# prip-lab/MSU-LatentAFIS

Hardware: AMD Instinct MI355X
Metric: latent queries/sec vs 100k rolled gallery (higher is better)
Workload: dtype f32

## Files before the change

### msu-latentafis_amd/csrc/graph.hip

```cpp
#include "afis_device.h"
#include <type_traits>
#include "atan2f_libm.h"
#include "graph_arith.h"
#include "stdsort_order.h"

namespace afis {

#define AFIS_PI 3.1415926

#if defined(AFIS_PHASE_TIMING) && !defined(AFIS_GRAPH_PAIRS_UNIT)
__device__ u64 g_graph_phase[16];
#define GPH_INIT() u64 gph_t0 = __builtin_readcyclecounter()
#define GPH(i) do { if (threadIdx.x == 0) { const u64 t1_ = __builtin_readcyclecounter(); sm.ph[(i)] += t1_ - gph_t0; gph_t0 = t1_; } } while (0)
#define GPH_T0() const u64 gph_k0 = __builtin_readcyclecounter()
#define GPH_K(i) do { if (threadIdx.x == 0) sm.ph[(i)] += __builtin_readcyclecounter() - gph_k0; } while (0)
#define GPH_ZERO() do { if (threadIdx.x < 16) sm.ph[threadIdx.x] = 0; WSYNC(); } while (0)
#define GPH_FLUSH() do { WSYNC(); if (threadIdx.x < 16 && sm.ph[threadIdx.x]) atomicAdd(&g_graph_phase[threadIdx.x], sm.ph[threadIdx.x]); } while (0)
#else
#define GPH_INIT() do {} while (0)
#define GPH(i) do {} while (0)
#define GPH_T0() do {} while (0)
#define GPH_K(i) do {} while (0)
#define GPH_ZERO() do {} while (0)
#define GPH_FLUSH() do {} while (0)
#endif

__device__ __forceinline__ u64 g_make_key(float v, int idx) { return rank_composite(rank_key(v), (uint32_t)idx); }
__device__ __forceinline__ int g_wave_popc(bool p) { return __popcll(__ballot(p)); }
__device__ __forceinline__ int g_lane_prefix(u64 mask) { return __builtin_amdgcn_mbcnt_hi((uint32_t)(mask >> 32), __builtin_amdgcn_mbcnt_lo((uint32_t)mask, 0)); }
#define WSYNC() __syncthreads()

__device__ __forceinline__ int g_wave_max(int x)
{
    x = max(x, __builtin_amdgcn_update_dpp(0, x, 0xB1, 0xf, 0xf, false));
    x = max(x, __builtin_amdgcn_update_dpp(0, x, 0x4E, 0xf, 0xf, false));
    x = max(x, __builtin_amdgcn_update_dpp(0, x, 0x124, 0xf, 0xf, false));
    x = max(x, __builtin_amdgcn_update_dpp(0, x, 0x128, 0xf, 0xf, false));
    x = max(x, __builtin_amdgcn_update_dpp(x, x, 0x142, 0xa, 0xf, false));
    x = max(x, __builtin_amdgcn_update_dpp(x, x, 0x143, 0xc, 0xf, false));
    return __builtin_amdgcn_readlane(x, 63);
}

__device__ __forceinline__ uint32_t g_wave_max_u32(uint32_t x) { return (uint32_t)g_wave_max((int)(x ^ 0x80000000u)) ^ 0x80000000u; }
__device__ __forceinline__ uint32_t g_wave_min_u32(uint32_t x) { return ~g_wave_max_u32(~x); }

__device__ __forceinline__ int g_wave_sum(int x)
{
    x += __builtin_amdgcn_update_dpp(0, x, 0xB1, 0xf, 0xf, false);
    x += __builtin_amdgcn_update_dpp(0, x, 0x4E, 0xf, 0xf, false);
    x += __builtin_amdgcn_update_dpp(0, x, 0x124, 0xf, 0xf, false);
    x += __builtin_amdgcn_update_dpp(0, x, 0x128, 0xf, 0xf, false);
    x += __builtin_amdgcn_update_dpp(0, x, 0x142, 0xa, 0xf, false);
    x += __builtin_amdgcn_update_dpp(0, x, 0x143, 0xc, 0xf, false);
    return __builtin_amdgcn_readlane(x, 63);
}

typedef __amdgpu_buffer_rsrc_t SlabBuf;
typedef uint32_t v4u __attribute__((ext_vector_type(4)));
__device__ __forceinline__ SlabBuf g_slab_buf(unsigned char* base, uint32_t bytes) { return __builtin_amdgcn_make_buffer_rsrc(base, 0, (int)bytes, 0x00020000); }

struct Pt { int lx, ly, rx, ry; };
__device__ __forceinline__ int2 pack_xy(int lx, int ly, int rx, int ry) { return make_int2((lx & 0xffff) | (ly << 16), (rx & 0xffff) | (ry << 16)); }
__device__ __forceinline__ Pt unpack_xy(int2 v) { Pt p; p.lx = (int)(short)v.x; p.ly = v.x >> 16; p.rx = (int)(short)v.y; p.ry = v.y >> 16; return p; }

template <int N, bool OWN> struct SimStore { float simv[N]; };
template <int N> struct SimStore<N, false> {};

#ifndef AFIS_MINU_ALIAS
#define AFIS_MINU_ALIAS 1
#endif
constexpr int kSortShort = 48;
template <int NMAX_, bool OWN_SIM_>
struct __attribute__((aligned(16))) WaveSmem : SimStore<NMAX_, OWN_SIM_> {
    static constexpr int NMAX = NMAX_;
    static constexpr bool OWN_SIM = OWN_SIM_;
    static constexpr bool ALIAS_ORI = NMAX_ > 128 || AFIS_MINU_ALIAS;
    static constexpr int W = (NMAX + 31) / 32;
    static constexpr int N4 = (NMAX + 3) / 4 * 4;
    static constexpr int U = (NMAX + 63) / 64;
    float b[N4];
    union {
        float cc[N4];
        struct { short order[NMAX]; short sel[NMAX]; } os;
    } y;
    short li[NMAX], ri[NMAX];
    int2 xy[NMAX];
    union {
        uint32_t hb[NMAX][W];
        struct { uint32_t keys[N4]; short te[NMAX], targ[NMAX]; } pick;
        uint32_t s7key[NMAX > 128 ? 256 : 1];
    };
    union {
        uint32_t cnt[128];
        u64 keys[kSortShort];
        struct { float lo[ALIAS_ORI ? 1 : NMAX], ro[ALIAS_ORI ? 1 : NMAX]; } s;
    } x;
#ifdef AFIS_PHASE_TIMING
    u64 ph[16];
#endif
};
template <class SM> __device__ __forceinline__ int l_row(int v) { if constexpr (SM::OWN_SIM) return v; else return v & 1023; }
template <class SM> __device__ __forceinline__ int r_pt(int v) { if constexpr (SM::OWN_SIM) return v; else return v & 1023; }
__device__ __forceinline__ int tex_slot_of(int li, int ri) { return ((li >> 10) & 31) | (((ri >> 10) & 31) << 5); }
__device__ __forceinline__ short tex_pack_l(int row, int slot) { return (short)(row | ((slot & 31) << 10)); }
__device__ __forceinline__ short tex_pack_r(int pt, int slot) { return (short)(pt | ((slot >> 5) << 10)); }
template <class SM>
__device__ __forceinline__ float list_sim(const SM& sm, const float* __restrict__ ext, int t)
{
    if constexpr (SM::OWN_SIM) return sm.simv[t];
    else return ext[tex_slot_of(sm.li[t], sm.ri[t])];
}

__device__ __forceinline__ int next_task(int32_t* ctr)
{
    int t;
    unsigned long long saved;
    asm volatile("s_mov_b64 %1, exec\n\t"
                 "s_mov_b64 exec, 1\n\t"
                 "global_atomic_add %0, %2, %3, %4 sc0\n\t"
                 "s_waitcnt vmcnt(0)\n\t"
                 "s_mov_b64 exec, %1"
                 : "=&v"(t), "=&s"(saved) : "v"(0), "v"(1), "s"(ctr) : "memory");
    return __builtin_amdgcn_readfirstlane(t);
}

template <class SM, int ref_tie>
__device__ __forceinline__ void sort_scores(SM& sm, int num, double thr)
{
    const int lane = threadIdx.x;
    constexpr int U = SM::U;
    uint32_t* const s_cnt = sm.x.cnt;
    uint32_t* const s_gkey = reinterpret_cast<uint32_t*>(sm.y.cc);
    uint32_t* const s_key = s_gkey;
    uint32_t m32[U]; int r[U];
    if (num <= kSortShort) {
        const u64 mine = lane < num ? g_make_key(sm.b[lane], lane) : 0ull;
        if (lane < num) sm.x.keys[lane] = mine;
        WSYNC();
        int rr = 0;
        for (int k = 0; k < num; ++k) rr += sm.x.keys[k] > mine;
        if (ref_tie && num > 16) {
            int gg = 0;
            for (int k = 0; k < num; ++k) gg += (uint32_t)(sm.x.keys[k] >> 32) > (uint32_t)(mine >> 32);
            const bool tied = lane < num && gg != rr && !((double)sm.b[lane] < thr);
            if (__ballot(tied) != 0ull) {
                constexpr int kOrd = kSortShort / 2;
                uint32_t* const k32 = s_gkey + kOrd;
                static_assert(SM::N4 >= kOrd + 2 * kSortShort, "no room in cc for the keys and the stack of the std::sort restatement");
                WSYNC();
                if (lane < num) { k32[lane] = (uint32_t)(mine >> 32); sm.y.os.order[lane] = (short)lane; }
                WSYNC();
                if (lane == 0) stdsort_prefix<uint16_t>(reinterpret_cast<uint16_t*>(sm.y.os.order), num, num, k32, reinterpret_cast<int*>(k32 + kSortShort));
                WSYNC();
                return;
            }
        }
        WSYNC();
        if (lane < num) sm.y.os.order[rr] = (short)lane;
        WSYNC();
        return;
    }
    uint32_t kmin = 0xffffffffu, kmax = 0u;
#pragma unroll
    for (int u = 0; u < U; ++u) {
        const int t = lane + 64 * u;
        m32[u] = t < num ? rank_key(sm.b[t]) : 0u;
        if (t < num) { kmin = min(kmin, m32[u]); kmax = max(kmax, m32[u]); }
    }
#pragma unroll
    for (int off = 32; off >= 1; off >>= 1) { kmin = min(kmin, (uint32_t)__shfl_xor((int)kmin, off)); kmax = max(kmax, (uint32_t)__shfl_xor((int)kmax, off)); }
    const uint32_t span = kmax - kmin;
    const int sh = max(0, 26 - __clz((int)(span | 1u)));
    int bin[U];
// ... 150 lines not shown
    if (LOOKUP) {
        const int dx1 = abs(a.lx - o.lx), dx2 = abs(a.rx - o.rx), dy1 = abs(a.ly - o.ly), dy2 = abs(a.ry - o.ry);
        ok = !((dx1 >= kDistN) | (dx2 >= kDistN) | (dy1 >= kDistN) | (dy2 >= kDistN));
        d1 = sqrt_rn_pos((float)(256 * (dx1 * dx1 + dy1 * dy1)));
        d2 = sqrt_rn_pos((float)(256 * (dx2 * dx2 + dy2 * dy2)));
        (void)table;
    } else {
        const float dx1 = (float)(a.lx - o.lx), dx2 = (float)(a.rx - o.rx), dy1 = (float)(a.ly - o.ly), dy2 = (float)(a.ry - o.ry);
        const float p = dx1 * dx1, q = dy1 * dy1, r = dx2 * dx2, s = dy2 * dy2;
        d1 = sqrt_rn_pos(p + q);
        d2 = sqrt_rn_pos(r + s);
    }
    dist = fabsf(d1 - d2);
    return ok;
}
template <bool LOOKUP>
__device__ __forceinline__ bool pair_compatible(const Pt& a, const Pt& o, const float* __restrict__ table)
{
    float s1, s2; bool ok = true;
    if (LOOKUP) {
        const int dx1 = abs(a.lx - o.lx), dx2 = abs(a.rx - o.rx), dy1 = abs(a.ly - o.ly), dy2 = abs(a.ry - o.ry);
        ok = !((dx1 >= kDistN) | (dx2 >= kDistN) | (dy1 >= kDistN) | (dy2 >= kDistN));
        s1 = (float)(256 * (dx1 * dx1 + dy1 * dy1)); s2 = (float)(256 * (dx2 * dx2 + dy2 * dy2));
    } else {
        const float dx1 = (float)(a.lx - o.lx), dx2 = (float)(a.rx - o.rx), dy1 = (float)(a.ly - o.ly), dy2 = (float)(a.ry - o.ry);
        const float p = dx1 * dx1, q = dy1 * dy1, r = dx2 * dx2, s = dy2 * dy2;
        s1 = p + q; s2 = r + s;
    }
    const float d1 = __builtin_amdgcn_sqrtf(s1), d2 = __builtin_amdgcn_sqrtf(s2);
    const float dist = fabsf(d1 - d2);
    const float slack = fmaxf(d1, d2) * 4.76837158e-7f;
    if (fabsf(dist - 30.0f) > slack) return ok && dist < 30.0f;
    float exact;
    pair_dist<LOOKUP>(a, o, table, exact);
    return ok && exact < 30.0f;
}
template <bool RANGE_TEST>
__device__ __forceinline__ bool tex_pair_dist(int2 a, int2 o, float& dist)
{
    float n1, n2;
    pair_n(a, o, n1, n2);
    dist = 16.0f * fabsf(sqrt_rn_int(n1) - sqrt_rn_int(n2));
    return RANGE_TEST ? tex_in_range(a, o) : true;
}
template <bool RANGE_TEST>
__device__ __forceinline__ bool tex_pair_compatible(int2 a, int2 o)
{
    float n1, n2;
    pair_n(a, o, n1, n2);
    const bool ok = RANGE_TEST ? tex_in_range(a, o) : true;
    return pair_compatible_n<true>(n1, n2) && ok;
}

__device__ __forceinline__ float minu_pair_dist(int2 a, int2 o)
{
    float n1, n2;
    pair_n(a, o, n1, n2);
    return fabsf(sqrt_rn_int(n1) - sqrt_rn_int(n2));
}
__device__ __forceinline__ bool minu_pair_compatible(int2 a, int2 o)
{
    float n1, n2;
    pair_n(a, o, n1, n2);
    return pair_compatible_n<false>(n1, n2);
}

__device__ __forceinline__ float h_of_x(float x)
{
    const float q0 = x * 0.04f;
    const float r = fmaf(-q0, 25.0f, x);
    const float h = fmaf(r, 0.04f, q0);
    return __builtin_amdgcn_fmed3f(h, 0.0f, 1.0f);
}
__device__ __forceinline__ float h_value(float dist)
{
    const float x = 30.0f - dist;
    const float q0 = x * 0.04f;
    const float r = fmaf(-q0, 25.0f, x);
    const float h = fmaf(r, 0.04f, q0);
    return __builtin_amdgcn_fmed3f(h, 0.0f, 1.0f);
}

template <class SM, bool LOOKUP, int ITERS, int MODE, int REF_TIE>
__device__ int dist_filter(SM& sm, int num, const float* __restrict__ table, const float* __restrict__ ext, SlabBuf slab)
{
    constexpr bool fast = MODE > 0;
    constexpr bool range_test = MODE == 1;
    auto compat_fast = [](int2 a, int2 o) -> bool { if (LOOKUP) return tex_pair_compatible<range_test>(a, o); return minu_pair_compatible(a, o); };
    auto dist_fast = [](int2 a, int2 o) -> float { float d; if (LOOKUP) { tex_pair_dist<range_test>(a, o, d); return d; } return minu_pair_dist(a, o); };
    constexpr int U = SM::U, W = SM::W, NMAX = SM::NMAX;
    [[maybe_unused]] constexpr int PH = LOOKUP ? 8 : 0;
    GPH_INIT();
    const int lane = threadIdx.x;
    for (int i = lane; i < num * W; i += 64) sm.hb[i / W][i % W] = 0u;
    int2 me[U];
#pragma unroll
    for (int u = 0; u < U; ++u) {
        const int t = lane + 64 * u;
        if (t < SM::N4) { sm.b[t] = t < num ? list_sim(sm, ext, t) : 0.0f; sm.y.cc[t] = 0.0f; }
        me[u] = t < num ? sm.xy[t] : make_int2(0, 0);
    }
    WSYNC();
    const int half = num >> 1;
    const bool even = !(num & 1);
    uint32_t* const hb0 = &sm.hb[0][0];
    auto pair = [&](int2 own, int t, int k, int2 other) {
        if (fast ? compat_fast(own, other) : pair_compatible<LOOKUP>(unpack_xy(own), unpack_xy(other), table)) {
            atomicOr(hb0 + (t * W + (k >> 5)), 1u << (k & 31));
            atomicOr(hb0 + (__umul24(k, W) + (t >> 5)), 1u << (t & 31));
        }
    };
    const int tail0 = num & ~63, R = num - tail0;
    const bool grouped = R > 0 && R <= 32;
    const int n_wide = grouped ? tail0 : num;
    uint32_t kb[U];
    const uint32_t num8 = (uint32_t)num * 8u;
#pragma unroll
    for (int u = 0; u < U; ++u) { const int t = lane + 64 * u; kb[u] = t < num ? (uint32_t)t * 8u : 0u; }
#ifndef AFIS_PAIR_UNROLL
#define AFIS_PAIR_UNROLL 1
#endif
    constexpr int DU = fast ? AFIS_PAIR_UNROLL : 1;
    auto pair_loop = [&](auto ua_tag) {
    constexpr int UA = decltype(ua_tag)::value;
    for (int d = 1; d <= half; d += DU) {
        int2 other[DU][UA];
        int kk[DU][UA];
#pragma unroll
        for (int s2 = 0; s2 < DU; ++s2) {
#pragma unroll
            for (int u = 0; u < UA; ++u) {
                const uint32_t a = kb[u] + 8u;
                kb[u] = min(a, a - num8);
                other[s2][u] = *reinterpret_cast<const int2*>(reinterpret_cast<const char*>(sm.xy) + kb[u]);
                kk[s2][u] = (int)(kb[u] >> 3);
            }
        }
        __builtin_amdgcn_sched_barrier(0);
        if (fast) {
            float n1[DU][UA], n2[DU][UA]; bool hit[DU][UA], near[DU][UA]; bool any_near = false;
#pragma unroll
            for (int s2 = 0; s2 < DU; ++s2) {
#pragma unroll
                for (int u = 0; u < UA; ++u) {
                    pair_n(me[u], other[s2][u], n1[s2][u], n2[s2][u]);
                    hit[s2][u] = pair_compatible_t<LOOKUP>(n1[s2][u], n2[s2][u], near[s2][u]);
                    hit[s2][u] = hit[s2][u] | near[s2][u];
                }
            }
            (void)any_near;
#pragma unroll
            for (int s2 = 0; s2 < DU; ++s2) {
                const bool last = d + s2 == half && even;
#pragma unroll
                for (int u = 0; u < UA; ++u) {
                    const int t = lane + 64 * u, k = kk[s2][u];
                    bool ok = hit[s2][u] && t < n_wide && d + s2 <= half && !(last && t >= half);
                    if (LOOKUP && range_test) ok = ok && tex_in_range(me[u], other[s2][u]);
                    if constexpr (LOOKUP) {
                        const int ts = t < num ? t : 0;
                        atomicOr(hb0 + (ts * W + (k >> 5)), ok ? 1u << (k & 31) : 0u);
                        atomicOr(hb0 + (__umul24(k, W) + (ts >> 5)), ok ? 1u << (ts & 31) : 0u);
                    } else if (ok) {
                        atomicOr(hb0 + (t * W + (k >> 5)), 1u << (k & 31));
                        atomicOr(hb0 + (__umul24(k, W) + (t >> 5)), 1u << (t & 31));
                    }
                }
            }
        } else {
            const bool last = d == half && even;
#pragma unroll
            for (int u = 0; u < UA; ++u) {
                const int t = lane + 64 * u;
                if (t < n_wide && !(last && t >= half)) pair(me[u], t, kk[0][u], other[0][u]);
            }
        }
    }
    };
    const int n_blk = (n_wide + 63) >> 6;
    if (n_blk >= U) pair_loop(std::integral_constant<int, U>{});
    else if (U > 1 && n_blk == U - 1) pair_loop(std::integral_constant<int, (U > 1 ? U - 1 : 1)>{});
    else if (n_blk > 0) pair_loop(std::integral_constant<int, U>{});
    if (grouped) {
        const int sh = R <= 8 ? 3 : R <= 16 ? 4 : 5, RG = 1 << sh, dstep = 64 >> sh;
        const int r = lane & (RG - 1), t = tail0 + r;
        const bool row = r < R;
        const int2 own = row ? sm.xy[t] : make_int2(0, 0);
        int d = 1 + (lane >> sh);
        int k = t + d; k = k >= num ? k - num : k;
        for (int d0 = 1; d0 <= half; d0 += dstep) {
            if (row && d <= half && !(d == half && even && t >= half)) pair(own, t, k, sm.xy[k]);
            d += dstep; k += dstep; k = k >= num ? k - num : k;
        }
    }
    WSYNC();
    GPH(PH + 0);
    int myrow[U], trip[U], rlen[U];
    const int Wn = (num + 31) / 32;
    {
        int cnt[U];
#pragma unroll
        for (int u = 0; u < U; ++u) {
            const int t = lane + 64 * u;
            int c = -1;
            if (t < num) {
                c = 0; for (int w = 0; w < Wn; ++w) c += __popc(sm.hb[t][w]);
                sm.y.os.sel[t] = (short)c;
                c = min(c >> 2, 15);
            }
            cnt[u] = c;
        }
        int base = 0;
        for (int bk = 15; bk >= 0; --bk) {
#pragma unroll
            for (int u = 0; u < U; ++u) {
                const bool in = cnt[u] == bk;
                const u64 m = __ballot(in);
                if (in) sm.y.os.order[base + g_lane_prefix(m)] = (short)(lane + 64 * u);
                base += __popcll(m);
            }
        }
        WSYNC();
#pragma unroll
        for (int u = 0; u < U; ++u) {
            const int p = lane + 64 * u;
            myrow[u] = p < num ? (int)sm.y.os.order[p] : -1;
            rlen[u] = myrow[u] >= 0 ? (int)sm.y.os.sel[myrow[u]] : 0;
            trip[u] = g_wave_max(rlen[u]);
        }
        WSYNC();
        for (int t = num + lane; t < SM::N4; t += 64) sm.y.cc[t] = 0.0f;
    }
    int2 mine[U];
#pragma unroll
    for (int u = 0; u < U; ++u) mine[u] = myrow[u] >= 0 ? sm.xy[myrow[u]] : make_int2(0, 0);
    constexpr bool kFlat = NMAX > 128;
    constexpr int kSlabN = kFlat ? kTexSlabSteps : kMinuSlabSteps;
    static_assert(kSlabN % 4 == 0, "the read loop takes blocks of four steps");
    static_assert((size_t)U * kSlabN * 64 * 5 == (kFlat ? kTexSlabWgBytes : kMinuSlabWgBytes), "slab layout and the size the host allocates differ");
    constexpr int kSlabBlk = kSlabN / 4;
    constexpr uint32_t kSlabIdx0 = (uint32_t)U * kSlabN * 64 * 4;
    const uint32_t lane16 = (uint32_t)lane * 16u, lane4 = (uint32_t)lane * 4u;
    auto put_block = [&](int e, const float (&h)[4], uint32_t k4) {
        __builtin_amdgcn_raw_buffer_store_b128(v4u{__float_as_uint(h[0]), __float_as_uint(h[1]), __float_as_uint(h[2]), __float_as_uint(h[3])}, slab, lane16, e * 1024, 0);
        __builtin_amdgcn_raw_buffer_store_b32(k4, slab, lane4, (int)kSlabIdx0 + e * 256, 0);
    };
    auto get_block = [&](int e, v4u& h, uint32_t& k4) {
        h = __builtin_amdgcn_raw_buffer_load_b128(slab, lane16, e * 1024, 0);
        k4 = __builtin_amdgcn_raw_buffer_load_b32(slab, lane4, (int)kSlabIdx0 + e * 256, 0);
    };
    int cur_w[U]; uint32_t cur_bits[U];
#pragma unroll
    for (int u = 0; u < U; ++u) { cur_w[u] = 0; cur_bits[u] = 0u; }
    auto value = [&](int2 own, int k) -> float {
        float dist;
        if (fast && LOOKUP) {
            float n1, n2;
            pair_n(own, sm.xy[k], n1, n2);
            return h_of_x(fmaf(-16.0f, fabsf(sqrt_rn_int(n1) - sqrt_rn_int(n2)), 30.0f));
        }
        if (fast) dist = dist_fast(own, sm.xy[k]);
        else pair_dist<LOOKUP>(unpack_xy(own), unpack_xy(sm.xy[k]), table, dist);
        return h_value(dist);
    };
    for (int it = 0; it < ITERS; ++it) {
#pragma unroll
        for (int u = 0; u < U; ++u) {
            const int t = myrow[u];
            const uint32_t* hrow = sm.hb[t >= 0 ? t : 0];
            float acc = 0.0f;
            if (it == 0) {
                if (t >= 0) {
                    int w = 0;
                    uint32_t bits = hrow[0];
                    for (int n0 = 0; n0 < trip[u]; n0 += 4) {
                        if (n0 == kSlabN) { cur_w[u] = w; cur_bits[u] = bits; }
                        float h4[4] = {0.0f, 0.0f, 0.0f, 0.0f};
                        uint32_t k4 = 0u;
#pragma unroll
                        for (int j = 0; j < 4; ++j) {
                            if (n0 + j < trip[u]) {
                                while (bits == 0u && w + 1 < Wn) { ++w; bits = hrow[w]; }
                                const bool have = bits != 0u;
                                const int k = (w * 32 + __ffs(bits) - 1) & 255;
                                bits &= bits - 1;
                                const float h = value(mine[u], k);
                                h4[j] = h; k4 |= (uint32_t)k << (8 * j);
                                const float p = h * sm.b[k];
                                acc += have ? p : 0.0f;
                            }
                        }
                        if (n0 < kSlabN) put_block(u * kSlabBlk + (n0 >> 2), h4, k4);
                    }
                }
            } else {
                const int nS = min(trip[u], kSlabN);
                v4u hc = {0u, 0u, 0u, 0u}; uint32_t kc = 0u;
                if (nS > 0) get_block(u * kSlabBlk, hc, kc);
                for (int n0 = 0; n0 < nS; n0 += 4) {
                    const float hn[4] = {__uint_as_float(hc.x), __uint_as_float(hc.y), __uint_as_float(hc.z), __uint_as_float(hc.w)};
                    const uint32_t kn = kc;
                    if (n0 + 4 < nS) get_block(u * kSlabBlk + (n0 >> 2) + 1, hc, kc);
#pragma unroll
                    for (int j = 0; j < 4; ++j) {
                        const float p = hn[j] * sm.b[(kn >> (8 * j)) & 255u];
                        acc += n0 + j < rlen[u] ? p : 0.0f;
                    }
                }
                if (trip[u] > kSlabN) {
                    int w = cur_w[u];
                    uint32_t bits = cur_bits[u];
                    for (int n = kSlabN; n < trip[u]; ++n) {
                        while (bits == 0u && w + 1 < Wn) { ++w; bits = t >= 0 ? hrow[w] : 0u; }
                        const bool have = bits != 0u;
                        const int k = (w * 32 + __ffs(bits) - 1) & 255;
                        bits &= bits - 1;
                        const float p = value(mine[u], k) * sm.b[k];
                        acc += have ? p : 0.0f;
                    }
                }
            }
            if (t >= 0) sm.y.cc[t] = acc;
        }
        WSYNC();
        const float sum = seq_sum(sm, num);
        const float scale = (float)(1.0 / ((double)sum + 0.00001));
#pragma unroll
        for (int u = 0; u < U; ++u) { const int t = lane + 64 * u; if (t < num) sm.b[t] = sm.y.cc[t] * scale; }
        WSYNC();
    }
    GPH(PH + 1);
    sort_scores<SM, REF_TIE>(sm, num, 0.0001);
    GPH(PH + 2);
    const int nsel = greedy(sm, num, 0.0001, [&sm, table, dist_fast](int a, int o) {
        if (!((sm.hb[a][o >> 5] >> (o & 31)) & 1u)) return false;
        float dist;
        if (fast) dist = dist_fast(sm.xy[a], sm.xy[o]);
        else pair_dist<LOOKUP>(unpack_xy(sm.xy[a]), unpack_xy(sm.xy[o]), table, dist);
        return !((double)h_value(dist) < 0.00001);
    });
    compact(sm, nsel);
    GPH(PH + 3);
    return nsel;
}

__device__ __forceinline__ float adjust_angle(float angle)
{
    if ((double)angle > AFIS_PI) angle = (float)((double)angle - 2 * AFIS_PI);
    else if ((double)angle < -AFIS_PI) angle = (float)((double)angle + 2 * AFIS_PI);
    return angle;
}
__device__ __forceinline__ float fold_pi(float d)
{
    if ((double)d > AFIS_PI) d = (float)(2 * AFIS_PI - (double)d);
    return d;
}
__device__ __forceinline__ float atan2_f32(float y, float x) { return afis_atan2f_libm(y, x); }

__device__ __forceinline__ bool angle_compatible(const Pt& p1, float lo1, float ro1, const Pt& p2, float lo2, float ro2)
{
    float angle_1 = adjust_angle(lo1 - lo2);
    float angle_2 = adjust_angle(ro1 - ro2);
    float angle_diff = fold_pi(fabsf(angle_1 - angle_2));
    if ((double)angle_diff > AFIS_PI / 4.) return false;
    const float dx_1 = (float)(p1.lx - p2.lx), dy_1 = (float)(p1.ly - p2.ly);
    const float line_angle_1 = -atan2_f32(dy_1, dx_1);
    angle_1 = adjust_angle(lo1 - line_angle_1);
    const float dx_2 = (float)(p1.rx - p2.rx), dy_2 = (float)(p1.ry - p2.ry);
    const float line_angle_2 = -atan2_f32(dy_2, dx_2);
    angle_2 = adjust_angle(ro1 - line_angle_2);
    angle_diff = fold_pi(fabsf(angle_1 - angle_2));
    if ((double)angle_diff > AFIS_PI / 6.) return false;
    angle_1 = adjust_angle(lo2 - line_angle_1);
    angle_2 = adjust_angle(ro2 - line_angle_2);
    angle_diff = fold_pi(fabsf(angle_1 - angle_2));
    if ((double)angle_diff > AFIS_PI / 6.) return false;
    return true;
}

template <class SM, int REF_TIE>
__device__ int angle_filter(SM& sm, int num, const float* __restrict__ lori, const float* __restrict__ rori)
{
    constexpr int W = SM::W;
    [[maybe_unused]] constexpr int PH = SM::NMAX > 128 ? 8 : 0;
    GPH_INIT();
    const int lane = threadIdx.x;
    if constexpr (SM::ALIAS_ORI) {
        for (int t = lane; t < num; t += 64) { sm.b[t] = lori[l_row<SM>(sm.li[t])]; sm.y.cc[t] = rori[r_pt<SM>(sm.ri[t])]; }
        for (int i = lane; i < num * W; i += 64) sm.hb[i / W][i % W] = 0u;
    } else {
        for (int t = lane; t < num; t += 64) { sm.x.s.lo[t] = lori[l_row<SM>(sm.li[t])]; sm.x.s.ro[t] = rori[r_pt<SM>(sm.ri[t])]; }
        for (int i = lane; i < num * W; i += 64) sm.hb[i / W][i % W] = 0u;
        const float s0 = (float)(1.0 / num);
        for (int t = lane; t < SM::N4; t += 64) { sm.b[t] = t < num ? s0 : 0.0f; sm.y.cc[t] = 0.0f; }
    }
    WSYNC();
    const int half = num >> 1;
    const bool even = !(num & 1);
    auto pair = [&](int t, int k) {
        const int i = t < k ? t : k, j = t < k ? k : t;
        bool ok;
        if constexpr (SM::ALIAS_ORI) ok = angle_compatible(unpack_xy(sm.xy[i]), sm.b[i], sm.y.cc[i], unpack_xy(sm.xy[j]), sm.b[j], sm.y.cc[j]);
        else ok = angle_compatible(unpack_xy(sm.xy[i]), sm.x.s.lo[i], sm.x.s.ro[i], unpack_xy(sm.xy[j]), sm.x.s.lo[j], sm.x.s.ro[j]);
        if (ok) {
            atomicOr(&sm.hb[i][j >> 5], 1u << (j & 31));
            atomicOr(&sm.hb[j][i >> 5], 1u << (i & 31));
        }
    };
    const int tail0 = num & ~63, R = num - tail0;
    const bool grouped = R > 0 && R <= 32;
    const int n_wide = grouped ? tail0 : num;
    for (int d = 1; n_wide > 0 && d <= half; ++d) {
        for (int t = lane; t < n_wide; t += 64) {
            if (d == half && even && t >= half) continue;
            int k = t + d; if (k >= num) k -= num;
            pair(t, k);
        }
    }
    if (grouped) {
        const int sh = R <= 8 ? 3 : R <= 16 ? 4 : 5, RG = 1 << sh, dstep = 64 >> sh;
        const int r = lane & (RG - 1), t = tail0 + r;
        int d = 1 + (lane >> sh);
        int k = t + d; k = k >= num ? k - num : k;
        for (int d0 = 1; d0 <= half; d0 += dstep) {
            if (r < R && d <= half && !(d == half && even && t >= half)) pair(t, k);
            d += dstep; k += dstep; k = k >= num ? k - num : k;
        }
    }
    WSYNC();
    if constexpr (SM::ALIAS_ORI) {
        const float s0 = (float)(1.0 / num);
        for (int t = lane; t < SM::N4; t += 64) { sm.b[t] = t < num ? s0 : 0.0f; sm.y.cc[t] = 0.0f; }
        WSYNC();
    }
    GPH(PH + 4);
    for (int it = 0; it < 5; ++it) {
        for (int t = lane; t < num; t += 64) {
            float s1 = 0.0f;
            for (int w = 0; w < (num + 31) / 32; ++w) {
                uint32_t bits = sm.hb[t][w];
                while (bits) { const int k = w * 32 + __ffs(bits) - 1; bits &= bits - 1; s1 += sm.b[k]; }
            }
            sm.y.cc[t] = s1;
        }
        WSYNC();
        float sum = seq_sum(sm, num);
        sum = (float)(1.0 / ((double)sum + 0.00001));
        for (int t = lane; t < num; t += 64) sm.b[t] = sm.y.cc[t] * sum;
        WSYNC();
    }
    GPH(PH + 5);
    sort_scores<SM, REF_TIE>(sm, num, 0.001);
    const int nsel = greedy(sm, num, 0.001, [&sm](int a, int o) { return (sm.hb[a][o >> 5] >> (o & 31)) & 1u; });
    compact(sm, nsel);
    GPH(PH + 6);
    return nsel;
}

template <class SM, bool LOOKUP, int ITERS, int REF_TIE>
__device__ __forceinline__ float graph_score(SM& sm, int num, const float* __restrict__ table, const float* __restrict__ lori,
                                             const float* __restrict__ rori, const float* __restrict__ ext, SlabBuf slab, int& n_survivors, int stop_after = 2, int mode = 0)
{
    n_survivors = num;
    if (stop_after == 0) return 0.0f;
    if (mode == 2 && LOOKUP) num = dist_filter<SM, LOOKUP, ITERS, 2, REF_TIE>(sm, num, table, ext, slab);
    else if (mode >= 1) num = dist_filter<SM, LOOKUP, ITERS, 1, REF_TIE>(sm, num, table, ext, slab);
    else num = dist_filter<SM, LOOKUP, ITERS, 0, REF_TIE>(sm, num, table, ext, slab);
    n_survivors = num;
    if (mode >= 1) {
        for (int t = threadIdx.x; t < num; t += 64) {
            const int2 v = sm.xy[t];
            int lx, ly, rx, ry;
            unpack_h2(v.x, lx, ly); unpack_h2(v.y, rx, ry);
            sm.xy[t] = pack_xy(lx, ly, rx, ry);
        }
        WSYNC();
    }
    if (stop_after == 1) return 0.0f;
    n_survivors = 0;
    if (num < 2) return 0.0f;
    num = angle_filter<SM, REF_TIE>(sm, num, lori, rori);
    n_survivors = num;
    for (int t = threadIdx.x; t < num; t += 64) sm.b[t] = list_sim(sm, ext, t);
    WSYNC();
    float score = 0.0f;
    for (int i = 0; i < num; ++i) score += sm.b[i];
    return score;
}

struct GraphTap { MinuCand* out; int32_t* n; int stage; };
template <class SM>
__device__ __forceinline__ void tap_write(const GraphTap& tap, const SM& sm, const float* __restrict__ ext, long long task, int n, int cap)
{
    for (int t = threadIdx.x; t < n; t += 64) { MinuCand c; c.sim = list_sim(sm, ext, t); c.li = l_row<SM>(sm.li[t]); c.ri = r_pt<SM>(sm.ri[t]); tap.out[(size_t)task * cap + t] = c; }
    if (threadIdx.x == 0) tap.n[task] = n;
}

#ifndef AFIS_TEX_WAVES
#define AFIS_TEX_WAVES 4
#endif
typedef WaveSmem<kTopTex, false> TexSmem;
static_assert(sizeof(TexSmem) <= 10240, "a texture list's LDS exceeds a sixteenth of a CU's: two of the CU's 16 wave slots would stay empty");
static_assert(sizeof(TexSmem::pick) <= sizeof(TexSmem::hb), "S7's scratch exceeds the bit rows it borrows");
constexpr int kTexRegs = (kTexMax + 63) / 64;
constexpr int kTexFast = 256;
constexpr int kTexFastRegs = kTexFast / 64;

__device__ __forceinline__ const int32_t* pair_tab_of() { return nullptr; }
__device__ __forceinline__ const int32_t* pair_tab_of(const int32_t* tab) { return tab; }
template <int REF_TIE, class... TAB>
__global__ __launch_bounds__(64) __attribute__((amdgpu_waves_per_eu(AFIS_TEX_WAVES, AFIS_TEX_WAVES))) void k_graph_texture(QueryDev q, GalleryDev g, const float* __restrict__ table_dist,
                                                      const float* __restrict__ rm_val, const int32_t* __restrict__ rm_arg,
                                                      const float* __restrict__ rm_cv, const int32_t* __restrict__ rm_n,
                                                      float* __restrict__ parts, unsigned char* slab_all, GraphTap tap, TAB... tab)
{
    constexpr bool PAIRS = sizeof...(TAB) != 0;
    const int32_t* const ptab = pair_tab_of(tab...);
    __shared__ TexSmem sm;
    const SlabBuf slab = g_slab_buf(slab_all + (size_t)blockIdx.x * kTexSlabWgBytes, (uint32_t)kTexSlabWgBytes);
    const int lane = threadIdx.x;
    GPH_ZERO();
    int n_tasks;
    if constexpr (PAIRS) n_tasks = ptab[0]; else n_tasks = q.nq * g.G;
    for (;;) {
        const int task = next_task(g.task_ctr + 0);
        if (task >= n_tasks) break;
        GPH_T0();
        int qi, gi;
        if constexpr (PAIRS) { qi = ptab[1 + 2 * task]; gi = ptab[2 + 2 * task]; }
        else { qi = task / g.G; gi = task - qi * g.G; }
        const int l0 = q.lt_off[qi], n_lt = q.lt_off[qi + 1] - l0;
        const int r0 = g.tex_off[gi], n_rt = g.tex_off[gi + 1] - r0;
        float* out = parts + (size_t)task * 4 + 3;
        if (n_lt <= 0 || n_rt <= 0) { if (lane == 0) { *out = 0.0f; if (tap.out) tap.n[task] = -1; } continue; }
        const size_t o = (size_t)task * q.lt_pad;
        int num;
        if (n_lt > kTopTex) {
            const bool compact = rm_n != nullptr;
            const int n_in = compact ? rm_n[task] : n_lt;
            if (compact && n_in >= kTopTex && n_in <= kTexFast) {
                uint32_t key[kTexFastRegs]; int arg[kTexFastRegs];
                uint32_t kmin = 0xffffffffu, kmax = 0u;
#pragma unroll
                for (int u = 0; u < kTexFastRegs; ++u) {
                    const int e = u * 64 + lane;
                    const bool in = e < n_in;
                    key[u] = in ? rank_key(rm_cv[o + e]) : 0u;
                    arg[u] = in ? rm_arg[o + e] : 0;
                    kmax = max(kmax, key[u]);
                    if (in) kmin = min(kmin, key[u]);
                }
                kmin = g_wave_min_u32(kmin); kmax = g_wave_max_u32(kmax);
                const int shift = max(0, 27 - __clz((int)((kmax - kmin) >> 1) | 1));
                uint32_t* const s_cnt = reinterpret_cast<uint32_t*>(sm.b);
                uint32_t* const s_gkey = sm.s7key;
                static_assert(TexSmem::N4 >= 128 && sizeof(sm.s7key) >= (size_t)kTexFast * 4 && sizeof(sm.s7key) <= sizeof(sm.hb), "the counting arrays of the compact S7 exceed their buffers");
                int bin[kTexFastRegs], r[kTexFastRegs];
#pragma unroll
                for (int u = 0; u < kTexFastRegs; ++u) bin[u] = min((int)((key[u] - kmin) >> shift), 63);
                s_cnt[lane] = 0u;
                WSYNC();
#pragma unroll
                for (int u = 0; u < kTexFastRegs; ++u) if (u * 64 + lane < n_in) atomicAdd(&s_cnt[bin[u]], 1u);
                WSYNC();
                {
                    const int own = (int)s_cnt[lane];
                    int suf = own;
#pragma unroll
                    for (int off = 1; off < 64; off <<= 1) { const int v = __shfl_down(suf, off); if (lane + off < 64) suf += v; }
                    WSYNC();
                    s_cnt[lane] = (uint32_t)(suf - own); s_cnt[64 + lane] = (uint32_t)(suf - own);
                }
                WSYNC();
#pragma unroll
                for (int u = 0; u < kTexFastRegs; ++u) if (u * 64 + lane < n_in) s_gkey[atomicAdd(&s_cnt[bin[u]], 1u)] = key[u];
                WSYNC();
                int rsum = 0;
#pragma unroll
                for (int u = 0; u < kTexFastRegs; ++u) {
                    r[u] = 0;
                    if (u * 64 + lane < n_in) {
                        const int lo = (int)s_cnt[64 + bin[u]], hi = (int)s_cnt[bin[u]];
                        int c = lo;
                        for (int k = lo; k < hi; ++k) c += s_gkey[k] > key[u];
                        r[u] = c; rsum += c;
                    }
                }
                if (g_wave_sum(rsum) != n_in * (n_in - 1) / 2) {
                    WSYNC();
#pragma unroll
                    for (int u = 0; u < kTexFastRegs; ++u) if (u * 64 + lane < n_in) s_gkey[u * 64 + lane] = key[u];
                    WSYNC();
                    u64 mine[kTexFastRegs];
#pragma unroll
                    for (int u = 0; u < kTexFastRegs; ++u) { mine[u] = ((u64)key[u] << 32) | (uint32_t)(~(uint32_t)(u * 64 + lane)); r[u] = 0; }
                    for (int k = 0; k < n_in; ++k) {
                        const u64 kk = ((u64)s_gkey[k] << 32) | (uint32_t)(~(uint32_t)k);
#pragma unroll
                        for (int u = 0; u < kTexFastRegs; ++u) r[u] += kk > mine[u];
                    }
                }
#pragma unroll
                for (int u = 0; u < kTexFastRegs; ++u) {
                    const int e = u * 64 + lane;
                    if (e < n_in && r[u] < kTopTex) { sm.li[r[u]] = tex_pack_l(arg[u] & 0xffff, e); sm.ri[r[u]] = tex_pack_r(arg[u] >> 16, e); }
                }
                num = kTopTex;
            } else {
                const int n_regs = (n_in + 63) >> 6;
                uint32_t key[kTexRegs]; int arg[kTexRegs];
#pragma unroll
                for (int u = 0; u < kTexRegs; ++u) {
                    const int e = u * 64 + lane;
                    const bool in = e < n_in;
                    key[u] = 0u; arg[u] = 0;
                    if (u < n_regs) {
                        key[u] = in ? rank_key(compact ? rm_cv[o + e] : rm_val[o + e]) : 0u;
                        arg[u] = in ? rm_arg[o + e] : 0;
                    }
                }
                uint32_t T = 0;
                for (int bit = 31; bit >= 0; --bit) {
                    const uint32_t cand = T | (1u << bit);
                    int c = 0;
#pragma unroll
                    for (int u = 0; u < kTexRegs; ++u) if (u < n_regs) c += g_wave_popc(key[u] >= cand);
                    if (c >= kTopTex) { T = cand; if (c == kTopTex) break; }
                }
                int n_gt = 0;
#pragma unroll
                for (int u = 0; u < kTexRegs; ++u) if (u < n_regs) n_gt += g_wave_popc(key[u] > T);
                const int need = kTopTex - n_gt;
                int base_gt = 0, base_eq = 0;
                uint32_t* const key32 = sm.pick.keys;
#pragma unroll
                for (int u = 0; u < kTexRegs; ++u) {
                    if (u < n_regs) {
                        const int e = u * 64 + lane;
                        const bool gt = key[u] > T, eq = key[u] == T;
                        const u64 mg = __ballot(gt), me = __ballot(eq);
                        int pos = -1;
                        if (gt) pos = base_gt + g_lane_prefix(mg);
                        else if (eq) { const int r = base_eq + g_lane_prefix(me); if (r < need) pos = n_gt + r; }
                        if (pos >= 0) { key32[pos] = key[u]; sm.pick.te[pos] = tex_pack_l(compact ? arg[u] & 0xffff : e, e); sm.pick.targ[pos] = tex_pack_r(compact ? arg[u] >> 16 : arg[u], e); }
                        base_gt += __popcll(mg); base_eq += __popcll(me);
                    }
                }
                WSYNC();
                num = kTopTex;
                uint32_t m32[TexSmem::U]; int r[TexSmem::U];
                uint32_t* const s_cnt = reinterpret_cast<uint32_t*>(sm.b);
                uint32_t* const s_gkey = reinterpret_cast<uint32_t*>(sm.y.cc);
                int dmax = 0;
#pragma unroll
                for (int u = 0; u < TexSmem::U; ++u) {
                    const int t = lane + 64 * u;
                    m32[u] = t < num ? key32[t] : T;
                    dmax = max(dmax, (int)((m32[u] - T) >> 1));
                }
                dmax = g_wave_max(dmax);
                const int shift = max(0, 27 - __clz(dmax | 1));
                int bin[TexSmem::U];
#pragma unroll
                for (int u = 0; u < TexSmem::U; ++u) bin[u] = min((int)((m32[u] - T) >> shift), 63);
                s_cnt[lane] = 0u;
                WSYNC();
#pragma unroll
                for (int u = 0; u < TexSmem::U; ++u) if (lane + 64 * u < num) atomicAdd(&s_cnt[bin[u]], 1u);
                WSYNC();
                {
                    const int own = (int)s_cnt[lane];
                    int suf = own;
#pragma unroll
                    for (int off = 1; off < 64; off <<= 1) { const int v = __shfl_down(suf, off); if (lane + off < 64) suf += v; }
                    WSYNC();
                    s_cnt[lane] = (uint32_t)(suf - own); s_cnt[64 + lane] = (uint32_t)(suf - own);
                }
                WSYNC();
#pragma unroll
                for (int u = 0; u < TexSmem::U; ++u) if (lane + 64 * u < num) s_gkey[atomicAdd(&s_cnt[bin[u]], 1u)] = m32[u];
                WSYNC();
#pragma unroll
                for (int u = 0; u < TexSmem::U; ++u) {
                    r[u] = 0;
                    if (lane + 64 * u < num) {
                        const int lo = (int)s_cnt[64 + bin[u]], hi = (int)s_cnt[bin[u]];
                        int c = lo;
                        for (int k = lo; k < hi; ++k) c += s_gkey[k] > m32[u];
                        r[u] = c;
                    }
                }
                int rsum = 0;
#pragma unroll
                for (int u = 0; u < TexSmem::U; ++u) rsum += r[u];
                if (g_wave_sum(rsum) != kTopTex * (kTopTex - 1) / 2) {
                    u64 mine[TexSmem::U];
#pragma unroll
                    for (int u = 0; u < TexSmem::U; ++u) { const int t = lane + 64 * u; mine[u] = t < num ? ((u64)key32[t] << 32) | (uint32_t)(~(uint32_t)(sm.pick.te[t] & 1023)) : 0ull; r[u] = 0; }
                    for (int k = 0; k < num; ++k) {
                        const u64 kk = ((u64)key32[k] << 32) | (uint32_t)(~(uint32_t)(sm.pick.te[k] & 1023));
#pragma unroll
                        for (int u = 0; u < TexSmem::U; ++u) r[u] += kk > mine[u];
                    }
                }
#pragma unroll
                for (int u = 0; u < TexSmem::U; ++u) {
                    const int t = lane + 64 * u;
                    if (t < num) { sm.li[r[u]] = sm.pick.te[t]; sm.ri[r[u]] = sm.pick.targ[t]; }
                }
            }
        } else {
            num = n_lt;
            for (int t = lane; t < num; t += 64) { sm.li[t] = tex_pack_l(t, t); sm.ri[t] = tex_pack_r(rm_n ? rm_arg[o + t] >> 16 : rm_arg[o + t], t); }
        }
        WSYNC();
        int out_of_range = 0, not_small = 0;
        short2 lp4[TexSmem::U], rp4[TexSmem::U];
#pragma unroll
        for (int u = 0; u < TexSmem::U; ++u) {
            const int t = lane + 64 * u;
            lp4[u] = make_short2(0, 0); rp4[u] = make_short2(0, 0);
            if (t < num) {
                lp4[u] = q.lt_xy[l0 + (sm.li[t] & 1023)]; rp4[u] = g.tex_xy[r0 + (sm.ri[t] & 1023)];
                out_of_range |= (lp4[u].x | lp4[u].y | rp4[u].x | rp4[u].y) & ~2047;
                not_small |= ((unsigned)lp4[u].x > 49u) | ((unsigned)lp4[u].y > 49u) | ((unsigned)rp4[u].x > 49u) | ((unsigned)rp4[u].y > 49u);
            }
        }
        const int mode = __ballot(out_of_range != 0) != 0ull ? 0 : (__ballot(not_small != 0) == 0ull ? 2 : 1);
#pragma unroll
        for (int u = 0; u < TexSmem::U; ++u) {
            const int t = lane + 64 * u;
            if (t < num) sm.xy[t] = mode ? make_int2(pack_h2(lp4[u].x, lp4[u].y), pack_h2(rp4[u].x, rp4[u].y)) : pack_xy(lp4[u].x, lp4[u].y, rp4[u].x, rp4[u].y);
        }
        WSYNC();
        GPH_K(15);
        int n_surv;
        const float* const row_max = (rm_n ? rm_cv : rm_val) + o;
        const float score = graph_score<TexSmem, true, 3, REF_TIE>(sm, num, table_dist, q.lt_ori + l0, g.tex_ori + r0, row_max, slab, n_surv, tap.out ? tap.stage : 2, mode);
        if (lane == 0) *out = score;
        if (tap.out) tap_write(tap, sm, row_max, task, n_surv, kTopTex);
        WSYNC();
    }
    GPH_FLUSH();
}

#ifndef AFIS_GRAPH_PAIRS_UNIT
hipError_t launch_graph_texture(const QueryDev& q, const GalleryDev& g, const float* table_dist,
                                const float* rm_val, const int32_t* rm_arg, const float* rm_cv, const int32_t* rm_n, float* parts, void* slab, size_t slab_bytes, MinuCand* tap_out, int32_t* tap_n, int tap_stage, hipStream_t stream)
{
    const long long n_tasks = (long long)q.nq * g.G;
    if (n_tasks <= 0) return hipSuccess;
    if (n_tasks > 0x7ffffff0LL || !g.task_ctr) return hipErrorInvalidValue;
    const int grid = graph_texture_grid(n_tasks);
    if (!slab || slab_bytes < (size_t)grid * kTexSlabWgBytes) return hipErrorInvalidValue;
    hipError_t e0 = hipMemsetAsync(g.task_ctr + 0, 0, 4, stream);
    if (e0 != hipSuccess) return e0;
    const GraphTap tap{tap_out, tap_n, tap_stage & 255};
    if ((tap_stage >> 8) & 1) hipLaunchKernelGGL(k_graph_texture<1>, dim3(grid), dim3(64), 0, stream, q, g, table_dist, rm_val, rm_arg, rm_cv, rm_n, parts, (unsigned char*)slab, tap);
    else hipLaunchKernelGGL(k_graph_texture<0>, dim3(grid), dim3(64), 0, stream, q, g, table_dist, rm_val, rm_arg, rm_cv, rm_n, parts, (unsigned char*)slab, tap);
    return hipGetLastError();
}
#else
hipError_t launch_graph_texture_pairs(const QueryDev& q, const GalleryDev& g, const int32_t* pair_tab, int n_pairs, const float* table_dist, const float* rm_val, const int32_t* rm_arg,
                                      float* parts, void* slab, size_t slab_bytes, int s89_tie_order, hipStream_t stream)
{
    if (n_pairs <= 0) return hipSuccess;
    if (!g.task_ctr || !pair_tab || !rm_val || !rm_arg || !parts) return hipErrorInvalidValue;
    const int grid = graph_texture_grid(n_pairs);
    if (!slab || slab_bytes < (size_t)grid * kTexSlabWgBytes) return hipErrorInvalidValue;
    const hipError_t e0 = hipMemsetAsync(g.task_ctr + 0, 0, 4, stream);
    if (e0 != hipSuccess) return e0;
    const GraphTap tap{nullptr, nullptr, 2};
    if (s89_tie_order) hipLaunchKernelGGL((k_graph_texture<1, const int32_t*>), dim3(grid), dim3(64), 0, stream, q, g, table_dist, rm_val, rm_arg, (const float*)nullptr, (const int32_t*)nullptr, parts, (unsigned char*)slab, tap, pair_tab);
    else hipLaunchKernelGGL((k_graph_texture<0, const int32_t*>), dim3(grid), dim3(64), 0, stream, q, g, table_dist, rm_val, rm_arg, (const float*)nullptr, (const int32_t*)nullptr, parts, (unsigned char*)slab, tap, pair_tab);
    return hipGetLastError();
}
#endif

typedef WaveSmem<kTopMinu, true> MinuGraphSmem;

#ifndef AFIS_MINU_WAVES
#define AFIS_MINU_WAVES 6
#endif
template <int REF_TIE, class... TAB>
__global__ __launch_bounds__(64) __attribute__((amdgpu_waves_per_eu(AFIS_MINU_WAVES, AFIS_MINU_WAVES))) void k_graph_minutiae(QueryDev q, GalleryDev g, const MinuCand* __restrict__ cands,
                                                       const int32_t* __restrict__ cand_n, float* __restrict__ parts,
                                                       short4* __restrict__ corr_out, int32_t* __restrict__ corr_n, unsigned char* slab_all, GraphTap tap, TAB... tab)
{
    constexpr bool PAIRS = sizeof...(TAB) != 0;
    const int32_t* const ptab = pair_tab_of(tab...);
    __shared__ MinuGraphSmem sm;
    const SlabBuf slab = g_slab_buf(slab_all + (size_t)blockIdx.x * kMinuSlabWgBytes, (uint32_t)kMinuSlabWgBytes);
    const int lane = threadIdx.x;
    GPH_ZERO();
    int n_tasks;
    if constexpr (PAIRS) n_tasks = 3 * ptab[0]; else n_tasks = q.nq * 3 * g.G;
    for (;;) {
        const int task = next_task(g.task_ctr + 1);
        if (task >= n_tasks) break;
        GPH_T0();
        int gi, qs;
        float* out;
        if constexpr (PAIRS) {
            const int p = task / 3, s = task - p * 3;
            qs = ptab[1 + 2 * p] * 3 + s; gi = ptab[2 + 2 * p];
            out = parts + (size_t)p * 4 + s;
        } else {
            gi = task % g.G;
            qs = task / g.G;
            const int qi = qs / 3, s = qs - qi * 3;
            out = parts + ((size_t)qi * g.G + gi) * 4 + s;
        }
        const int num = cand_n[task];
        if (num <= 0) { if (lane == 0) { *out = 0.0f; if (corr_n) corr_n[task] = 0; if (tap.out) tap.n[task] = -1; } continue; }
        const int l0 = q.lm_off[qs], r0 = g.minu_off[gi];
        const MinuCand* c = cands + (size_t)task * kTopMinu;
        int out_of_range = 0;
        short2 lp2[MinuGraphSmem::U], rp2[MinuGraphSmem::U];
#pragma unroll
        for (int u = 0; u < MinuGraphSmem::U; ++u) {
            const int t = lane + 64 * u;
// ... 155 lines not shown
```

Baseline: 54.76.

## Pair slab passes in dist_filter, widen S7 bins, reuse selected sims

Later iterations of the flat dist_filter path now walk two row slots at once, interleaving their slab loads so the buffer reads overlap. The compact S7 top-k histogram grows from 64 to 256 bins, using vectorized uint4 counts in its own smem region, so each bin's linear rank scan gets shorter. The selected similarity values are written straight into sm.b, so the list_sim recompute is skipped when b_filled is set. These add register pressure and some complexity in the iteration loop.

```diff
diff --git a/msu-latentafis_amd/csrc/graph.hip b/msu-latentafis_amd/csrc/graph.hip
--- a/msu-latentafis_amd/csrc/graph.hip
+++ b/msu-latentafis_amd/csrc/graph.hip
@@ -88,7 +88,7 @@
     union {
         uint32_t hb[NMAX][W];
         struct { uint32_t keys[N4]; short te[NMAX], targ[NMAX]; } pick;
-        uint32_t s7key[NMAX > 128 ? 256 : 1];
+        struct { uint32_t gkey[NMAX > 128 ? 256 : 1]; uint32_t cnt[NMAX > 128 ? 512 : 1]; } s7;
     };
     union {
         uint32_t cnt[128];
@@ -405,7 +405,7 @@
 }
 
 template <class SM, bool LOOKUP, int ITERS, int MODE, int REF_TIE>
-__device__ int dist_filter(SM& sm, int num, const float* __restrict__ table, const float* __restrict__ ext, SlabBuf slab)
+__device__ int dist_filter(SM& sm, int num, const float* __restrict__ table, const float* __restrict__ ext, SlabBuf slab, bool b_filled = false)
 {
     constexpr bool fast = MODE > 0;
     constexpr bool range_test = MODE == 1;
@@ -420,7 +420,12 @@
 #pragma unroll
     for (int u = 0; u < U; ++u) {
         const int t = lane + 64 * u;
-        if (t < SM::N4) { sm.b[t] = t < num ? list_sim(sm, ext, t) : 0.0f; sm.y.cc[t] = 0.0f; }
+        if (t < SM::N4) {
+            bool have_b = false;
+            if constexpr (!SM::OWN_SIM) have_b = b_filled && t < num;
+            if (!have_b) sm.b[t] = t < num ? list_sim(sm, ext, t) : 0.0f;
+            sm.y.cc[t] = 0.0f;
+        }
         me[u] = t < num ? sm.xy[t] : make_int2(0, 0);
     }
     WSYNC();
@@ -587,12 +592,69 @@
         return h_value(dist);
     };
     for (int it = 0; it < ITERS; ++it) {
+        if constexpr (kFlat) if (it > 0) {
+            constexpr int GS = 2;
+            static_assert(U % GS == 0, "the passes are read in pairs");
+#pragma unroll
+            for (int g = 0; g < U / GS; ++g) {
+                float acc[GS]; int nS[GS]; v4u hc[GS]; uint32_t kc[GS];
+                int n_max = 0;
+#pragma unroll
+                for (int i = 0; i < GS; ++i) {
+                    const int u = i == 0 ? g : U - 1 - g;
+                    acc[i] = 0.0f; nS[i] = min(trip[u], kSlabN); n_max = max(n_max, nS[i]);
+                    hc[i] = v4u{0u, 0u, 0u, 0u}; kc[i] = 0u;
+                    if (nS[i] > 0) get_block(u * kSlabBlk, hc[i], kc[i]);
+                }
+                for (int n0 = 0; n0 < n_max; n0 += 4) {
+                    float hn[GS][4]; uint32_t kn[GS];
+#pragma unroll
+                    for (int i = 0; i < GS; ++i) {
+                        const int u = i == 0 ? g : U - 1 - g;
+                        hn[i][0] = __uint_as_float(hc[i].x); hn[i][1] = __uint_as_float(hc[i].y); hn[i][2] = __uint_as_float(hc[i].z); hn[i][3] = __uint_as_float(hc[i].w);
+                        kn[i] = kc[i];
+                        if (n0 + 4 < nS[i]) get_block(u * kSlabBlk + (n0 >> 2) + 1, hc[i], kc[i]);
+                    }
+#pragma unroll
+                    for (int i = 0; i < GS; ++i) {
+                        const int u = i == 0 ? g : U - 1 - g;
+                        if (n0 < nS[i]) {
+#pragma unroll
+                            for (int j = 0; j < 4; ++j) {
+                                const float p = hn[i][j] * sm.b[(kn[i] >> (8 * j)) & 255u];
+                                acc[i] += n0 + j < rlen[u] ? p : 0.0f;
+                            }
+                        }
+                    }
+                }
+#pragma unroll
+                for (int i = 0; i < GS; ++i) {
+                    const int u = i == 0 ? g : U - 1 - g;
+                    const int t = myrow[u];
+                    if (trip[u] > kSlabN) {
+                        const uint32_t* hrow = sm.hb[t >= 0 ? t : 0];
+                        int w = cur_w[u];
+                        uint32_t bits = cur_bits[u];
+                        for (int n = kSlabN; n < trip[u]; ++n) {
+                            while (bits == 0u && w + 1 < Wn) { ++w; bits = t >= 0 ? hrow[w] : 0u; }
+                            const bool have = bits != 0u;
+                            const int k = (w * 32 + __ffs(bits) - 1) & 255;
+                            bits &= bits - 1;
+                            const float p = value(mine[u], k) * sm.b[k];
+                            acc[i] += have ? p : 0.0f;
+                        }
+                    }
+                    if (t >= 0) sm.y.cc[t] = acc[i];
+                }
+            }
+        }
+        if (!kFlat || it == 0) {
 #pragma unroll
         for (int u = 0; u < U; ++u) {
             const int t = myrow[u];
             const uint32_t* hrow = sm.hb[t >= 0 ? t : 0];
             float acc = 0.0f;
-            if (it == 0) {
+            if (kFlat || it == 0) {
                 if (t >= 0) {
                     int w = 0;
                     uint32_t bits = hrow[0];
@@ -644,6 +706,7 @@
                 }
             }
             if (t >= 0) sm.y.cc[t] = acc;
+        }
         }
         WSYNC();
         const float sum = seq_sum(sm, num);
@@ -782,13 +845,13 @@
 
 template <class SM, bool LOOKUP, int ITERS, int REF_TIE>
 __device__ __forceinline__ float graph_score(SM& sm, int num, const float* __restrict__ table, const float* __restrict__ lori,
-                                             const float* __restrict__ rori, const float* __restrict__ ext, SlabBuf slab, int& n_survivors, int stop_after = 2, int mode = 0)
+                                             const float* __restrict__ rori, const float* __restrict__ ext, SlabBuf slab, int& n_survivors, int stop_after = 2, int mode = 0, bool b_filled = false)
 {
     n_survivors = num;
     if (stop_after == 0) return 0.0f;
-    if (mode == 2 && LOOKUP) num = dist_filter<SM, LOOKUP, ITERS, 2, REF_TIE>(sm, num, table, ext, slab);
-    else if (mode >= 1) num = dist_filter<SM, LOOKUP, ITERS, 1, REF_TIE>(sm, num, table, ext, slab);
-    else num = dist_filter<SM, LOOKUP, ITERS, 0, REF_TIE>(sm, num, table, ext, slab);
+    if (mode == 2 && LOOKUP) num = dist_filter<SM, LOOKUP, ITERS, 2, REF_TIE>(sm, num, table, ext, slab, b_filled);
+    else if (mode >= 1) num = dist_filter<SM, LOOKUP, ITERS, 1, REF_TIE>(sm, num, table, ext, slab, b_filled);
+    else num = dist_filter<SM, LOOKUP, ITERS, 0, REF_TIE>(sm, num, table, ext, slab, b_filled);
     n_survivors = num;
     if (mode >= 1) {
         for (int t = threadIdx.x; t < num; t += 64) {
@@ -858,41 +921,48 @@
         if (n_lt <= 0 || n_rt <= 0) { if (lane == 0) { *out = 0.0f; if (tap.out) tap.n[task] = -1; } continue; }
         const size_t o = (size_t)task * q.lt_pad;
         int num;
+        bool b_filled = false;
         if (n_lt > kTopTex) {
             const bool compact = rm_n != nullptr;
             const int n_in = compact ? rm_n[task] : n_lt;
             if (compact && n_in >= kTopTex && n_in <= kTexFast) {
-                uint32_t key[kTexFastRegs]; int arg[kTexFastRegs];
+                uint32_t key[kTexFastRegs]; int arg[kTexFastRegs]; float val[kTexFastRegs];
                 uint32_t kmin = 0xffffffffu, kmax = 0u;
 #pragma unroll
                 for (int u = 0; u < kTexFastRegs; ++u) {
                     const int e = u * 64 + lane;
                     const bool in = e < n_in;
-                    key[u] = in ? rank_key(rm_cv[o + e]) : 0u;
+                    val[u] = in ? rm_cv[o + e] : 0.0f;
+                    key[u] = in ? rank_key(val[u]) : 0u;
                     arg[u] = in ? rm_arg[o + e] : 0;
                     kmax = max(kmax, key[u]);
                     if (in) kmin = min(kmin, key[u]);
                 }
                 kmin = g_wave_min_u32(kmin); kmax = g_wave_max_u32(kmax);
-                const int shift = max(0, 27 - __clz((int)((kmax - kmin) >> 1) | 1));
-                uint32_t* const s_cnt = reinterpret_cast<uint32_t*>(sm.b);
-                uint32_t* const s_gkey = sm.s7key;
-                static_assert(TexSmem::N4 >= 128 && sizeof(sm.s7key) >= (size_t)kTexFast * 4 && sizeof(sm.s7key) <= sizeof(sm.hb), "the counting arrays of the compact S7 exceed their buffers");
+                constexpr int kS7Bins = 256;
+                const int shift = max(0, 25 - __clz((int)((kmax - kmin) >> 1) | 1));
+                uint32_t* const s_cnt = sm.s7.cnt;
+                uint32_t* const s_gkey = sm.s7.gkey;
+                static_assert(sizeof(sm.s7.gkey) >= (size_t)kTexFast * 4 && sizeof(sm.s7.cnt) == (size_t)kS7Bins * 8 && kS7Bins == 4 * 64 && sizeof(sm.s7) <= sizeof(sm.hb) && offsetof(TexSmem, s7.cnt) % 16 == 0,
+                              "the counting arrays of the compact S7 exceed their buffers");
                 int bin[kTexFastRegs], r[kTexFastRegs];
 #pragma unroll
-                for (int u = 0; u < kTexFastRegs; ++u) bin[u] = min((int)((key[u] - kmin) >> shift), 63);
-                s_cnt[lane] = 0u;
+                for (int u = 0; u < kTexFastRegs; ++u) bin[u] = min((int)((key[u] - kmin) >> shift), kS7Bins - 1);
+                *reinterpret_cast<uint4*>(s_cnt + 4 * lane) = make_uint4(0u, 0u, 0u, 0u);
                 WSYNC();
 #pragma unroll
                 for (int u = 0; u < kTexFastRegs; ++u) if (u * 64 + lane < n_in) atomicAdd(&s_cnt[bin[u]], 1u);
                 WSYNC();
                 {
-                    const int own = (int)s_cnt[lane];
+                    const uint4 c = *reinterpret_cast<const uint4*>(s_cnt + 4 * lane);
+                    const int own = (int)(c.x + c.y + c.z + c.w);
                     int suf = own;
 #pragma unroll
                     for (int off = 1; off < 64; off <<= 1) { const int v = __shfl_down(suf, off); if (lane + off < 64) suf += v; }
+                    uint4 st;
+                    st.w = (uint32_t)(suf - own); st.z = st.w + c.w; st.y = st.z + c.z; st.x = st.y + c.y;
                     WSYNC();
-                    s_cnt[lane] = (uint32_t)(suf - own); s_cnt[64 + lane] = (uint32_t)(suf - own);
+                    *reinterpret_cast<uint4*>(s_cnt + 4 * lane) = st; *reinterpret_cast<uint4*>(s_cnt + kS7Bins + 4 * lane) = st;
                 }
                 WSYNC();
 #pragma unroll
@@ -903,7 +973,7 @@
                 for (int u = 0; u < kTexFastRegs; ++u) {
                     r[u] = 0;
                     if (u * 64 + lane < n_in) {
-                        const int lo = (int)s_cnt[64 + bin[u]], hi = (int)s_cnt[bin[u]];
+                        const int lo = (int)s_cnt[kS7Bins + bin[u]], hi = (int)s_cnt[bin[u]];
                         int c = lo;
                         for (int k = lo; k < hi; ++k) c += s_gkey[k] > key[u];
                         r[u] = c; rsum += c;
@@ -926,8 +996,9 @@
 #pragma unroll
                 for (int u = 0; u < kTexFastRegs; ++u) {
                     const int e = u * 64 + lane;
-                    if (e < n_in && r[u] < kTopTex) { sm.li[r[u]] = tex_pack_l(arg[u] & 0xffff, e); sm.ri[r[u]] = tex_pack_r(arg[u] >> 16, e); }
-                }
+                    if (e < n_in && r[u] < kTopTex) { sm.li[r[u]] = tex_pack_l(arg[u] & 0xffff, e); sm.ri[r[u]] = tex_pack_r(arg[u] >> 16, e); sm.b[r[u]] = val[u]; }
+                }
+                b_filled = true;
                 num = kTopTex;
             } else {
                 const int n_regs = (n_in + 63) >> 6;
@@ -1059,7 +1130,7 @@
         GPH_K(15);
         int n_surv;
         const float* const row_max = (rm_n ? rm_cv : rm_val) + o;
-        const float score = graph_score<TexSmem, true, 3, REF_TIE>(sm, num, table_dist, q.lt_ori + l0, g.tex_ori + r0, row_max, slab, n_surv, tap.out ? tap.stage : 2, mode);
+        const float score = graph_score<TexSmem, true, 3, REF_TIE>(sm, num, table_dist, q.lt_ori + l0, g.tex_ori + r0, row_max, slab, n_surv, tap.out ? tap.stage : 2, mode, b_filled);
         if (lane == 0) *out = score;
         if (tap.out) tap_write(tap, sm, row_max, task, n_surv, kTopTex);
         WSYNC();
```

Measured after the change: 55.15 (median of 6 runs). No clear change (+0.7%).
